# GalDude33/Fetal-MRI-Segmentation

Hardware: NVIDIA B200
Metric: U-Net train voxels/sec (higher is better)
Workload: dtype bf16

## Files before the change

fetal-mri-segmentation_b200/csrc/api.cu:

```cuda
#include <stdarg.h>

#include <algorithm>
#include <cmath>

#include "common.cuh"
#include <chrono>
#include <thread>

static thread_local char g_err[1024] = "";

void fm_set_error(const char* fmt, ...) {
  va_list ap;
  va_start(ap, fmt);
  vsnprintf(g_err, sizeof(g_err), fmt, ap);
  va_end(ap);
}
extern "C" const char* fm_last_error(void) { return g_err; }

extern "C" int fm_ctx_create(int device, fm_ctx** out) {
  FM_CHECK(out != nullptr, FM_EINVAL, "fm_ctx_create: out is NULL");
  int count = 0;
  FM_CUDA(cudaGetDeviceCount(&count));
  FM_CHECK(device >= 0 && device < count, FM_EINVAL, "fm_ctx_create: device %d of %d", device, count);
  FM_CUDA(cudaSetDevice(device));
// ... 810 lines not shown
      if (d < D - 1) {
        FM_TRY(m->gPool[d].ensure((size_t)m->vox(d + 1) * cap * lb.cout));
        const Layer &da = L(m, "dec%da", d), &db = L(m, "dec%db", d);
        if (!da.up_coarse && !da.up_dgrad) FM_TRY(m->gUp[d].ensure(v * da.c1));
        if (m->deconvolution) FM_TRY(m->dcG.ensure(v * da.c1));
        FM_TRY(m->gSkip[d].ensure(v * da.c2));
        FM_TRY(m->gDecA[d].ensure(v * da.cout));
        FM_TRY(m->gDecB[d].ensure(v * db.cout));
      }
    }
    m->train_alloc = true;
  }
  m->cap = cap;
  return FM_OK;
}

static int conv_fwd(fm_model* m, const Layer& l, const bf16* x1, const bf16* x2, bf16* y, int B, int relu = 1) {
  fm_ctx* ctx = m->ctx;
  const Dims5 d = m->dims(l.level, l.cout, B);
  const float* bias = m->params + l.b_off;
  if (l.march_f)
    return k_conv3d_march(ctx, x1, x2, l.w_mf[0], l.w_mf[1], bias, y, nullptr, B, d.X, d.Y, d.Z, l.c1, l.c2, l.cout, relu,
                          l.cout, 0, reproducible_pass(m));
  if (conv_tc_supported(l.c1, l.c2, l.cout, l.k))
    return k_conv3d_tc_fprop(ctx, x1, x2, l.w_f, bias, y, nullptr, B, d.X, d.Y, d.Z, l.c1, l.c2, l.cout,
                             l.k, relu, l.cout, 0);
  return k_conv3d_simt_fprop(ctx, x1, 0, x2, l.w_f, bias, y, nullptr, B, d.X, d.Y, d.Z, l.c1, l.c2,
                             l.cout, l.k, relu, nullptr);
}

static int bn_block_fwd(fm_model* m, const Layer& l, const void* x1, int x1_f32, const bf16* x2, bf16* y, int B) {
  fm_ctx* ctx = m->ctx;
  const int li = (int)(&l - &m->layers[0]);
  const Layer &nl = m->layers[li + 1], &ml = m->layers[li + 2];
  const Dims5 d = m->dims(l.level, l.cout, B);
  bf16* raw = m->train_pass ? m->bnRawL[li + 1].p : m->bnRaw.p;
  if (x1_f32)
    FM_TRY(k_conv3d_simt_fprop(ctx, x1, 1, nullptr, l.w_f, m->params + l.b_off, raw, nullptr, B, d.X, d.Y, d.Z, l.c1, 0,
                               l.cout, l.k, 0, nullptr));
  else
    FM_TRY(conv_fwd(m, l, (const bf16*)x1, x2, raw, B, 0));
  return k_batchnorm_relu(ctx, raw, m->params + nl.w_off, m->params + nl.b_off, m->params + ml.w_off,
                          m->params + ml.b_off, y, B, m->vox(l.level), l.cout, m->bnScratch.p, m->bnScratch.n,
                          m->train_pass ? m->bnStatsL[li + 1].p : nullptr, m->train_pass ? 1 : 0);
}

// ... 136 lines not shown
      FM_TRY(k_conv3d_tc_wgrad(ctx, xs[s], dy, dw, B, d.X, d.Y, d.Z, cs[s], l.cin(), cofs, l.cout, l.k));
    else
      FM_TRY(k_conv3d_simt_wgrad(ctx, xs[s], 0, dy, dw, B, d.X, d.Y, d.Z, cs[s], l.cin(), cofs, l.cout,
                                 l.k));
    cofs += cs[s];
  }
  if (!bias_done) FM_TRY(k_bias_grad(ctx, dy, m->grads + l.b_off, d.voxels(), l.cout));
  return FM_OK;
}

static int conv_wgrad_source(fm_model* m, const Layer& l, int src, const bf16* x, const bf16* dy, int B) {
  return conv_wgrad(m, l, src == 0 ? x : nullptr, src == 1 ? x : nullptr, dy, B, src);
}

static int conv_dgrad(fm_model* m, const Layer& l, int src, const bf16* dy, const bf16* mask, bf16* dx,
                      int B) {
  fm_ctx* ctx = m->ctx;
  const Dims5 d = m->dims(l.level, l.cout, B);
  const int cs = src == 0 ? l.c1 : l.c2;
  const bf16* wd = src == 0 ? l.w_d0 : l.w_d1;
  if (l.march_d[src])
    return k_conv3d_march(ctx, dy, nullptr, l.w_md[src], nullptr, nullptr, dx, mask, B, d.X, d.Y, d.Z, l.cout, 0, cs, 0,
                          cs, 0, reproducible_pass(m));
  if (conv_tc_supported(l.cout, 0, cs, l.k))
    return k_conv3d_tc_fprop(ctx, dy, nullptr, wd, nullptr, dx, mask, B, d.X, d.Y, d.Z, l.cout, 0, cs, l.k,
                             0, cs, 0);
  return k_conv3d_simt_fprop(ctx, dy, 0, nullptr, wd, nullptr, dx, nullptr, B, d.X, d.Y, d.Z, l.cout, 0,
                             cs, l.k, 0, mask);
}

static int mark_layer_done(fm_model* m, const Layer& l) {
  const int i = (int)(&l - &m->layers[0]);
  FM_CUDA(cudaEventRecord(m->layer_done[i], m->ctx->stream));
  return FM_OK;
}

static int backward_isensee(fm_model* m, int B);

static int bn_block_bwd(fm_model* m, const Layer& l, const bf16* gy, const bf16* gy2, int B) {
  const int li = (int)(&l - &m->layers[0]);
  const Layer& nl = m->layers[li + 1];
  FM_TRY(k_batchnorm_relu_bwd(m->ctx, m->bnRawL[li + 1].p, m->bnStatsL[li + 1].p, m->params + nl.w_off,
                              m->params + nl.b_off, gy, gy2, m->bnGRaw.p, m->grads + nl.w_off, m->grads + nl.b_off, B,
                              m->vox(l.level), l.cout, m->bnScratch.p, m->bnScratch.n));
  FM_TRY(mark_layer_done(m, m->layers[li + 2]));
  return mark_layer_done(m, nl);
// ... 380 lines not shown
      FM_TRY(m->isLoc1[l].ensure(n));
      FM_TRY(m->isLoc2[l].ensure(n));
      if (l < m->nseg) FM_TRY(m->isSeg[l].ensure((size_t)B * m->vox(l)));
    }
  }
  m->cap = B;
  return FM_OK;
}

static int isensee_block(fm_model* m, const Layer& l, const Layer& nl, const bf16* x1, const bf16* x2, const bf16* add,
                         bf16* y, int B, const float* chan_scale = nullptr) {
  fm_ctx* ctx = m->ctx;
  const Dims5 d = m->dims(l.level, l.cout, B);
  const float* bias = m->params + l.b_off;
  const int li = (int)(&l - &m->layers[0]);
  bf16* raw = m->train_pass ? m->isRawL[li].p : m->isRaw.p;
  float* stats = m->train_pass ? m->isStatsL[li].p : nullptr;
  if (l.c1 == 1) {
    FM_TRY(k_conv3d_simt_fprop(ctx, x1, 1, nullptr, l.w_f, bias, raw, nullptr, B, d.X, d.Y, d.Z, 1, 0, l.cout, 3, 0,
                               nullptr));
  } else if (l.march_f) {
    FM_TRY(k_conv3d_march(ctx, x1, x2, l.w_mf[0], l.w_mf[1], bias, raw, nullptr, B, d.X, d.Y, d.Z, l.c1, l.c2, l.cout, 0,
                          l.cout, 0, reproducible_pass(m)));
  } else if (conv_tc_supported(l.c1, l.c2, l.cout, l.k)) {
    FM_TRY(k_conv3d_tc_fprop(ctx, x1, x2, l.w_f, bias, raw, nullptr, B, d.X, d.Y, d.Z, l.c1, l.c2, l.cout, l.k, 0,
                             l.cout, 0, l.stride, d.X * l.stride, d.Y * l.stride, m->pz == 2 ? d.Z * l.stride : d.Z));
  } else {
    FM_CHECK(l.stride == 1, FM_EINVAL, "isensee: strided conv %s has no fallback", l.name);
    FM_TRY(k_conv3d_simt_fprop(ctx, x1, 0, x2, l.w_f, bias, raw, nullptr, B, d.X, d.Y, d.Z, l.c1, l.c2, l.cout, l.k, 0,
                               nullptr));
  }
  return k_instnorm_lrelu(ctx, raw, m->params + nl.w_off, m->params + nl.b_off, add, y, B, m->vox(l.level), l.cout,
                          m->isScratch.p, m->isScratch.n, stats, chan_scale);
}

static int forward_isensee(fm_model* m, int B) {
  fm_ctx* ctx = m->ctx;
  const int D = m->depth();
  FM_TRY(refresh_packs(m));
  auto LI = [&](const char* fmt, int d) {
    char nm[32];
    snprintf(nm, sizeof(nm), fmt, d);
    return layer_index(m, nm);
  };
  const bf16* cur = nullptr;
  for (int l = 0; l < D; ++l) {
// ... 50 lines not shown
  const bf16* xs[2] = {x1, x2};
  const int cs[2] = {l.c1, l.c2};
  int cofs = 0;
  for (int s = 0; s < (l.c2 ? 2 : 1); ++s) {
    if (conv_wgrad_march_supported(d.X, d.Y, d.Z, cs[s], l.cout, l.k))
      FM_TRY(k_conv3d_wgrad_march(ctx, xs[s], dy, dw, B, d.X, d.Y, d.Z, cs[s], l.cin(), cofs, l.cout));
    else if (conv_tc_supported(cs[s], 0, l.cout, l.k))
      FM_TRY(k_conv3d_tc_wgrad(ctx, xs[s], dy, dw, B, d.X, d.Y, d.Z, cs[s], l.cin(), cofs, l.cout, l.k));
    else
      FM_TRY(k_conv3d_simt_wgrad(ctx, xs[s], 0, dy, dw, B, d.X, d.Y, d.Z, cs[s], l.cin(), cofs, l.cout, l.k));
    cofs += cs[s];
  }
  return FM_OK;
}

static int is_dgrad(fm_model* m, const Layer& l, int level, int src, const bf16* dy, bf16* dx, int B) {
  fm_ctx* ctx = m->ctx;
  const Dims5 d = m->dims(level, l.cout, B);
  const int cs = src == 0 ? l.c1 : l.c2;
  const bf16* wd = src == 0 ? l.w_d0 : l.w_d1;
  if (l.march_d[src])
    return k_conv3d_march(ctx, dy, nullptr, l.w_md[src], nullptr, nullptr, dx, nullptr, B, d.X, d.Y, d.Z, l.cout, 0, cs, 0,
                          cs, 0, reproducible_pass(m));
  if (conv_tc_supported(l.cout, 0, cs, l.k))
    return k_conv3d_tc_fprop(ctx, dy, nullptr, wd, nullptr, dx, nullptr, B, d.X, d.Y, d.Z, l.cout, 0, cs, l.k, 0, cs, 0);
  return k_conv3d_simt_fprop(ctx, dy, 0, nullptr, wd, nullptr, dx, nullptr, B, d.X, d.Y, d.Z, l.cout, 0, cs, l.k, 0,
                             nullptr);
}

static int is_block_bwd(fm_model* m, int li, const bf16* gy, const bf16* gy2, const float* chan_scale, int B) {
  const Layer &l = m->layers[li], &nl = m->layers[li + 1];
  FM_TRY(k_instnorm_lrelu_bwd(m->ctx, m->isRawL[li].p, m->isStatsL[li].p, m->params + nl.w_off, m->params + nl.b_off, gy,
                              gy2, chan_scale, m->gIsRaw.p, m->grads + nl.w_off, m->grads + nl.b_off, B, m->vox(l.level),
                              l.cout, m->isScratch.p, m->isScratch.n));
  FM_TRY(mark_layer_done(m, nl));
  return FM_OK;
}

static int backward_isensee(fm_model* m, int B) {
  fm_ctx* ctx = m->ctx;
  const int D = m->depth();
  const int64_t n0 = (int64_t)B * m->vox(0);
  auto LI = [&](const char* fmt, int d) {
    char nm[32];
    snprintf(nm, sizeof(nm), fmt, d);
    return layer_index(m, nm);
// ... 927 lines not shown
  OpScratch s(ctx);
  const size_t vox = (size_t)N * X * Y * Z;
  const int taps = kext_taps(ksize), Ct = C1 + C2;
  std::vector<float> packed((size_t)Cout * taps * Ct);
  keras_to_packed(w_keras, packed.data(), ksize, Ct, Cout);
  bf16 *dx1 = nullptr, *dx2 = nullptr, *dw = nullptr, *dy = nullptr;
  float* dbias = nullptr;
  FM_TRY(s.up_bf16(x, vox * C1, &dx1));
  if (C2 > 0) FM_TRY(s.up_bf16(x2, vox * C2, &dx2));
  FM_TRY(s.up_bf16(packed.data(), packed.size(), &dw));
  if (bias) FM_TRY(s.up_f32(bias, Cout, &dbias));
  FM_TRY(s.alloc(&dy, vox * Cout));
  if (impl == 2 || impl == 3) {
    FM_CHECK(conv_march_supported(X, Y, Z, C1, C2, Cout, ksize), FM_EINVAL, "march kernel does not cover this shape");
    bf16 *wm1 = nullptr, *wm2 = nullptr;
    FM_TRY(s.alloc(&wm1, (size_t)conv_march_pack_elems(C1, Cout)));
    FM_TRY(k_repack_march(ctx, dw, wm1, Cout, Ct, 0, C1, conv_march_kc(C1, C2, Cout, C1)));
    if (C2 > 0) {
      FM_TRY(s.alloc(&wm2, (size_t)conv_march_pack_elems(C2, Cout)));
      FM_TRY(k_repack_march(ctx, dw, wm2, Cout, Ct, C1, C2, conv_march_kc(C1, C2, Cout, C2)));
    }
    FM_TRY(k_conv3d_march(ctx, dx1, dx2, wm1, wm2, dbias, dy, nullptr, N, X, Y, Z, C1, C2, Cout, relu, Cout, 0,
                          impl != 3));
  } else if (impl == 0)
    FM_TRY(k_conv3d_tc_fprop(ctx, dx1, dx2, dw, dbias, dy, nullptr, N, X, Y, Z, C1, C2, Cout, ksize, relu,
                             Cout, 0));
  else
    FM_TRY(k_conv3d_simt_fprop(ctx, dx1, 0, dx2, dw, dbias, dy, nullptr, N, X, Y, Z, C1, C2, Cout, ksize,
                               relu, nullptr));
  return s.down_bf16(dy, vox * Cout, y);
}

extern "C" int fm_op_conv3d_dgrad(fm_ctx* ctx, int impl, const float* dy, const float* w_keras,
                                  const float* mask, int N, int X, int Y, int Z, int Cin, int Cout,
                                  float* dx) {
  FM_CHECK(ctx && dy && w_keras && dx, FM_EINVAL, "fm_op_conv3d_dgrad: NULL argument");
  FM_CUDA(cudaSetDevice(ctx->device));
  OpScratch s(ctx);
  const size_t vox = (size_t)N * X * Y * Z;
  const int ksize = 3, taps = 27;
  std::vector<float> packed((size_t)Cout * taps * Cin);
  keras_to_packed(w_keras, packed.data(), ksize, Cin, Cout);
  float* dwm = nullptr;
  bf16 *wd = nullptr, *ddy = nullptr, *dmask = nullptr, *ddx = nullptr;
  FM_TRY(s.up_f32(packed.data(), packed.size(), &dwm));
  FM_TRY(s.alloc(&wd, packed.size()));
  FM_TRY(k_repack_weights(ctx, dwm, nullptr, wd, nullptr, Cout, taps, Cin, 0));
  FM_TRY(s.up_bf16(dy, vox * Cout, &ddy));
  if (mask) FM_TRY(s.up_bf16(mask, vox * Cin, &dmask));
  FM_TRY(s.alloc(&ddx, vox * Cin));
  if (impl == 2 || impl == 3) {
    FM_CHECK(conv_march_supported(X, Y, Z, Cout, 0, Cin, ksize), FM_EINVAL, "march kernel does not cover this shape");
    bf16* wm = nullptr;
    FM_TRY(s.alloc(&wm, (size_t)conv_march_pack_elems(Cout, Cin)));
    FM_TRY(k_repack_march(ctx, wd, wm, Cin, Cout, 0, Cout, conv_march_kc(Cout, 0, Cin, Cout)));
    FM_TRY(k_conv3d_march(ctx, ddy, nullptr, wm, nullptr, nullptr, ddx, dmask, N, X, Y, Z, Cout, 0, Cin, 0, Cin, 0,
                          impl != 3));
  } else if (impl == 0)
    FM_TRY(k_conv3d_tc_fprop(ctx, ddy, nullptr, wd, nullptr, ddx, dmask, N, X, Y, Z, Cout, 0, Cin, ksize, 0,
                             Cin, 0));
  else
    FM_TRY(k_conv3d_simt_fprop(ctx, ddy, 0, nullptr, wd, nullptr, ddx, nullptr, N, X, Y, Z, Cout, 0, Cin,
                               ksize, 0, dmask));
  return s.down_bf16(ddx, vox * Cin, dx);
}

extern "C" int fm_op_conv3d_wgrad(fm_ctx* ctx, int impl, const float* x, const float* dy, int N, int X,
                                  int Y, int Z, int Cin, int Cout, float* dw_keras, float* dbias) {
  FM_CHECK(ctx && x && dy && dw_keras, FM_EINVAL, "fm_op_conv3d_wgrad: NULL argument");
  FM_CUDA(cudaSetDevice(ctx->device));
  OpScratch s(ctx);
  const size_t vox = (size_t)N * X * Y * Z;
  const int ksize = 3, taps = 27;
  bf16 *dx = nullptr, *ddy = nullptr;
  float *dw = nullptr, *db = nullptr;
  FM_TRY(s.up_bf16(x, vox * Cin, &dx));
  FM_TRY(s.up_bf16(dy, vox * Cout, &ddy));
  const size_t wn = (size_t)Cout * taps * Cin;
  FM_TRY(s.alloc(&dw, wn));
  FM_TRY(s.alloc(&db, Cout));
// ... 232 lines not shown
```

fetal-mri-segmentation_b200/csrc/common.cuh:

```cuda
#pragma once
#include <cuda.h>
#include <cuda_bf16.h>
#include <cuda_runtime.h>
#include <stdint.h>
#include <stdio.h>
#include <stdlib.h>
#include <string.h>

#include <string>
#include <vector>

#include "../../include/fetal_b200.h"

typedef __nv_bfloat16 bf16;

void fm_set_error(const char* fmt, ...);

#define FM_CUDA(expr)                                                                         \
  do {                                                                                        \
    cudaError_t _e = (expr);                                                                  \
    if (_e != cudaSuccess) {                                                                  \
      fm_set_error("%s:%d: %s -> %s", __FILE__, __LINE__, #expr, cudaGetErrorString(_e));     \
      return FM_ECUDA;                                                                        \
    }                                                                                         \
// ... 248 lines not shown
                    int C, double* sums, XentSpec xs = XentSpec());
int k_dice_finalize(fm_ctx*, int nblocks, double n_elems, double* sums);
int k_head_bwd(fm_ctx*, const bf16* x, const float* dz, const float* w, bf16* dx, float* dw,
               float* db, int64_t voxels, int C, int mode = 0, const float* t = nullptr, const double* sums = nullptr,
               XentSpec xs = XentSpec());
struct RepackDesc {
  int64_t w_off;
  int cout, taps, c1, c2;
  bf16 *wf, *wd0, *wd1, *mf0, *mf1, *md0, *md1;
  int kcf0, kcf1, kcd0, kcd1;
  int block0;
};
int k_repack_all(fm_ctx*, const float* params, const RepackDesc* table_dev, int nlayers, int total_blocks,
                 double total_weights);
int k_repack_weights(fm_ctx*, const float* w, bf16* w_f, bf16* w_d0, bf16* w_d1, int Cout, int taps,
                     int C1, int C2);

struct ConvTcPlan;
int conv_tc_supported(int C1, int C2, int Cout, int ksize);
int k_conv3d_tc_fprop(fm_ctx*, const bf16* x1, const bf16* x2, const bf16* w_packed,
                      const float* bias, bf16* y, const bf16* mask, int N, int X, int Y, int Z,
                      int C1, int C2, int Cout, int ksize, int relu, int out_C, int out_cofs, int stride = 1,
                      int Xin = 0, int Yin = 0, int Zin = 0);
int k_conv3d_tc_wgrad(fm_ctx*, const bf16* x, const bf16* dy, float* dw_packed, int N, int X, int Y,
                      int Z, int Cin, int Cin_total, int cin_ofs, int Cout, int ksize);
int conv_up_supported(int X, int Y, int Z, int Cc, int Cs, int Cout);
int k_repack_up(fm_ctx*, const float* w_master, bf16* w_up_f, bf16* w_up_d, int Cout, int Cc, int Ct);
struct RepackUpDesc {
  int64_t w_off;
  bf16 *wf, *wd;
  int cout, cc, ct, block0;
};
struct RepackUpTable {
  RepackUpDesc d[8];
  int n;
};
int k_repack_up_table(fm_ctx*, const float* params, const RepackUpTable& tab);
int k_conv3d_up_fprop(fm_ctx*, const bf16* coarse, const bf16* skip, const bf16* w_up, const bf16* w_packed,
                      const float* bias, bf16* y, int N, int X, int Y, int Z, int Cc, int Cs, int Cout, int relu);
int k_conv3d_up_dgrad(fm_ctx*, const bf16* dy, const bf16* w_up_d, bf16* dcoarse, const bf16* mask, int N, int X,
                      int Y, int Z, int Cout, int Cc);
int k_conv3d_up_wgrad(fm_ctx*, const bf16* coarse, const bf16* dy, float* dw_up, int N, int X, int Y, int Z, int Cc,
                      int Cout);
int k_fold_up_wgrad(fm_ctx*, const float* dw_up, float* dw_master, int Cout, int Cc, int Ct);

int conv_first_tc_supported(int X, int Y, int Z, int Cout);
// ... 16 lines not shown
```

fetal-mri-segmentation_b200/csrc/conv_tc.cu:

```cuda
#include <algorithm>

#include "tc_ptx.cuh"

namespace {

using namespace tcp;

constexpr int kTileM = 128;
constexpr int kThreadsTc = 192;
constexpr uint32_t kABytes = kTileM * 128;

struct alignas(64) FpropParams {
  CUtensorMap tmA[2];
  CUtensorMap tmW[2];
  int nsrc;
  int nchunks[2];
  int KC[2];
  int wcofs[2];
  int N, X, Y, Z;
  int bx, by, bz, tx, ty, tz;
  int m_tiles, n_tiles, block_n;
  int ksize, ntaps;
  int out_C, out_cofs;
  int relu;
  int stages;
  int stride;
  int stride_z;
  int pbx, pby, pbz;
  int upmode;
  int ntaps_s[2];
  int oX, oY, oZ;
  const float* bias;
  bf16* out;
  const bf16* mask;
};

__global__ void __launch_bounds__(kThreadsTc, 1) conv3d_tc_fprop_kernel(
    const __grid_constant__ FpropParams p) {
  extern __shared__ uint8_t smem_raw[];
  const uint32_t smem0 = (smem_u32(smem_raw) + 1023u) & ~1023u;
  const int warp = threadIdx.x >> 5, lane = threadIdx.x & 31;

  const uint32_t b_bytes = (uint32_t)p.block_n * 128u;
  const uint32_t stage_bytes = kABytes + b_bytes;
  const uint32_t bar0 = smem0 + (uint32_t)p.stages * stage_bytes;
  auto full_bar = [&](int s) { return bar0 + 8u * (uint32_t)s; };
  auto empty_bar = [&](int s) { return bar0 + 8u * (uint32_t)(p.stages + s); };
  auto tfull_bar = [&](int a) { return bar0 + 8u * (uint32_t)(2 * p.stages + a); };
  auto tempty_bar = [&](int a) { return bar0 + 8u * (uint32_t)(2 * p.stages + 2 + a); };
  const uint32_t tmem_slot = bar0 + 8u * (uint32_t)(2 * p.stages + 4);

  uint32_t tmem_cols = 32;
  while (tmem_cols < 2u * (uint32_t)p.block_n) tmem_cols <<= 1;

  if (warp == 0 && lane == 0) {
    for (int s = 0; s < p.nsrc; ++s) {
      prefetch_tmap(&p.tmA[s]);
      prefetch_tmap(&p.tmW[s]);
// ... 147 lines not shown
      int m = tile / p.n_tiles;
      int cls = 0;
      if (p.upmode == 1) {
        cls = m & 7;
        m >>= 3;
      }
      const int iz = m % p.tz;
      m /= p.tz;
      const int iy = m % p.ty;
      m /= p.ty;
      const int ix = m % p.tx;
      const int n = m / p.tx;
      int x = ix * p.bx + rx, y = iy * p.by + ry, z = iz * p.bz + rz;
      const bool valid = (x < p.X) && (y < p.Y) && (z < p.Z);
      if (p.upmode == 1) {
        x = 2 * x + (cls >> 2);
        y = 2 * y + ((cls >> 1) & 1);
        z = 2 * z + (cls & 1);
      }
      const int64_t v = (((int64_t)n * p.oX + x) * p.oY + y) * p.oZ + z;
      const int64_t off = v * p.out_C + p.out_cofs + n_tile * p.block_n;
      mbar_wait(tfull_bar(acc), acc_ph);
      tc_fence_after();
      const uint32_t taddr = tmem_base + ((uint32_t)(q * 32) << 16) + acc * (uint32_t)p.block_n;
      for (int c16 = 0; c16 < p.block_n / 16; ++c16) {
        uint32_t r[16];
        tmem_ld16(taddr + (uint32_t)c16 * 16u, r);
        tmem_ld_wait();
        if (valid) {
          float f[16];
#pragma unroll
          for (int j = 0; j < 16; ++j) f[j] = __uint_as_float(r[j]);
          if (p.bias != nullptr) {
            const float4* bp =
                reinterpret_cast<const float4*>(p.bias + n_tile * p.block_n + c16 * 16);
#pragma unroll
            for (int j = 0; j < 4; ++j) {
              const float4 b4 = __ldg(bp + j);
              f[4 * j] += b4.x;
              f[4 * j + 1] += b4.y;
              f[4 * j + 2] += b4.z;
              f[4 * j + 3] += b4.w;
            }
          }
          if (p.relu) {
#pragma unroll
            for (int j = 0; j < 16; ++j) f[j] = fmaxf(f[j], 0.f);
          }
          if (p.mask != nullptr) {
            const uint4* mp = reinterpret_cast<const uint4*>(p.mask + off + c16 * 16);
#pragma unroll
            for (int h = 0; h < 2; ++h) {
              const uint4 mv = __ldg(mp + h);
              const __nv_bfloat162* mh = reinterpret_cast<const __nv_bfloat162*>(&mv);
#pragma unroll
              for (int j = 0; j < 4; ++j) {
                const float2 mf = __bfloat1622float2(mh[j]);
                if (!(mf.x > 0.f)) f[8 * h + 2 * j] = 0.f;
                if (!(mf.y > 0.f)) f[8 * h + 2 * j + 1] = 0.f;
              }
            }
          }
          uint4 o[2];
          __nv_bfloat162* oh = reinterpret_cast<__nv_bfloat162*>(o);
#pragma unroll
          for (int j = 0; j < 8; ++j) oh[j] = __floats2bfloat162_rn(f[2 * j], f[2 * j + 1]);
          uint4* op = reinterpret_cast<uint4*>(p.out + off + c16 * 16);
          op[0] = o[0];
          op[1] = o[1];
        }
      }
      tc_fence_before();
      mbar_arrive(tempty_bar(acc));
    }
  }

  tc_fence_before();
  __syncthreads();
  if (warp == 1) {
    tc_fence_after();
    tmem_dealloc(tmem_base, tmem_cols);
  }
}

struct alignas(64) WgradParams {
  CUtensorMap tmX;
  CUtensorMap tmDY;
  int KC, NC;
  int g;
  int ngroups;
  int G;
  int n_gsub;
  int n_cchunks;
  int n_nblocks;
  int NB;
  int splits;
// ... 226 lines not shown
  FM_CHECK(r == CUDA_SUCCESS, FM_ECUDA, "cuTensorMapEncodeTiled(weights) failed: %d (Cout=%d taps=%d Ct=%d)",
           (int)r, Cout, taps, Ct);
  return FM_OK;
}

int pow2_ceil(int v) {
  int p = 1;
  while (p < v) p <<= 1;
  return p;
}

void choose_box(int X, int Y, int Z, int* bx, int* by, int* bz) {
  int z = std::min(kTileM, pow2_ceil(Z));
  int y = std::min(kTileM / z, pow2_ceil(Y));
  int x = kTileM / (z * y);
  *bz = z;
  *by = y;
  *bx = x;
}

bool chan_ok(int C) { return C > 0 && C % 16 == 0 && (C <= 64 ? (C == 16 || C == 32 || C == 64) : C % 64 == 0); }
int chunk_of(int C) { return std::min(C, 64); }


}

int conv_tc_supported(int C1, int C2, int Cout, int ksize) {
  if (!(ksize == 1 || ksize == 3 || ksize == 31)) return 0;
  if (!chan_ok(C1)) return 0;
  if (C2 != 0 && !chan_ok(C2)) return 0;
  if (!(Cout == 16 || Cout == 32 || Cout == 64 || (Cout >= 128 && Cout % 128 == 0))) return 0;
  return 1;
}

int k_conv3d_tc_fprop(fm_ctx* ctx, const bf16* x1, const bf16* x2, const bf16* w_packed,
                      const float* bias, bf16* y, const bf16* mask, int N, int X, int Y, int Z, int C1,
                      int C2, int Cout, int ksize, int relu, int out_C, int out_cofs, int stride, int Xin,
                      int Yin, int Zin) {
  FM_CHECK(stride == 1 || (stride == 2 && kext_xy(ksize) == 3 && C2 == 0), FM_EINVAL,
           "conv3d tc: stride %d unsupported", stride);
  const int stride_z = kext_z(ksize) == 1 ? 1 : stride;
  if (stride == 1) {
    Xin = X;
    Yin = Y;
    Zin = Z;
  }
  FM_CHECK(conv_tc_supported(C1, C2, Cout, ksize), FM_EINVAL,
           "conv3d tc: unsupported channels C1=%d C2=%d Cout=%d k=%d", C1, C2, Cout, ksize);
  FM_CHECK(out_C % 8 == 0 && out_cofs % 8 == 0, FM_EINVAL, "conv3d tc: output channel pitch/offset");
  FpropParams p;
  memset(&p, 0, sizeof(p));
  p.nsrc = C2 > 0 ? 2 : 1;
  p.N = N;
  p.X = X;
  p.Y = Y;
  p.Z = Z;
  choose_box(X, Y, Z, &p.bx, &p.by, &p.bz);
  p.tx = ceil_div(X, p.bx);
  p.ty = ceil_div(Y, p.by);
  p.tz = ceil_div(Z, p.bz);
  p.m_tiles = N * p.tx * p.ty * p.tz;
  p.block_n = std::min(Cout, 128);
  while (p.block_n > 32 && p.m_tiles * (Cout / p.block_n) * 2 <= ctx->num_sms) p.block_n /= 2;
  p.n_tiles = Cout / p.block_n;
  p.ksize = ksize;
  p.ntaps = kext_taps(ksize);
  p.out_C = out_C;
  p.out_cofs = out_cofs;
  p.relu = relu;
  p.bias = bias;
  p.out = y;
  p.mask = mask;
  p.stride = stride;
  p.stride_z = stride_z;
  p.upmode = 0;
  p.ntaps_s[0] = p.ntaps_s[1] = p.ntaps;
  p.oX = X;
  p.oY = Y;
  p.oZ = Z;
  {
    auto pb = [&](int out, int in, int k, int st) { return std::max((out - 1) * st + k - in, 0) / 2; };
    p.pbx = pb(X, Xin, kext_xy(ksize), stride);
    p.pby = pb(Y, Yin, kext_xy(ksize), stride);
    p.pbz = pb(Z, Zin, kext_z(ksize), stride_z);
  }
  const int Ct = C1 + C2;
// ... 4 lines not shown
    p.KC[s] = chunk_of(Cs[s]);
    p.nchunks[s] = Cs[s] / p.KC[s];
    p.wcofs[s] = cofs;
    FM_TRY(make_act_tmap(&p.tmA[s], xs[s], N, Xin, Yin, Zin, Cs[s], p.KC[s], p.bz, p.by, p.bx, stride, stride_z));
    FM_TRY(make_w_tmap(&p.tmW[s], w_packed, Cout, p.ntaps, Ct, p.KC[s], p.block_n));
    cofs += Cs[s];
  }
  const uint32_t stage_bytes = kABytes + (uint32_t)p.block_n * 128u;
  int stages = (kMaxDynSmem - 2048) / (int)stage_bytes;
  stages = std::max(2, std::min(stages, 8));
  p.stages = stages;
  const size_t smem = (size_t)stages * stage_bytes + 1024  + 256 ;
  static bool attr_set = false;
  if (!attr_set) {
    FM_CUDA(cudaFuncSetAttribute(conv3d_tc_fprop_kernel, cudaFuncAttributeMaxDynamicSharedMemorySize,
                                 kMaxDynSmem));
    attr_set = true;
  }
  const int grid = std::min(p.m_tiles * p.n_tiles, ctx->num_sms);
  const double vox = (double)N * X * Y * Z;
  ProfScope prof(ctx, mask != nullptr || bias == nullptr ? "conv3d_tc_dgrad" : "conv3d_tc_fprop",
                 2.0 * p.ntaps * Ct * Cout * vox, vox * (Ct + Cout) * 2.0);
  FM_CUDA(launch_pdl(conv3d_tc_fprop_kernel, dim3(grid), dim3(kThreadsTc), smem, ctx->stream, p));
  FM_LAUNCH_OK(ctx);
  return FM_OK;
}

namespace {

int launch_tc_fprop(fm_ctx* ctx, FpropParams& p, const char* name, double flops, double bytes) {
  const uint32_t stage_bytes = kABytes + (uint32_t)p.block_n * 128u;
  int stages = (kMaxDynSmem - 2048) / (int)stage_bytes;
  stages = std::max(2, std::min(stages, 8));
  p.stages = stages;
  const size_t smem = (size_t)stages * stage_bytes + 1024  + 256 ;
  static bool attr_set = false;
  if (!attr_set) {
    FM_CUDA(cudaFuncSetAttribute(conv3d_tc_fprop_kernel, cudaFuncAttributeMaxDynamicSharedMemorySize, kMaxDynSmem));
    attr_set = true;
  }
  const int grid = std::min(p.m_tiles * p.n_tiles, ctx->num_sms);
  ProfScope prof(ctx, name, flops, bytes);
  FM_CUDA(launch_pdl(conv3d_tc_fprop_kernel, dim3(grid), dim3(kThreadsTc), smem, ctx->stream, p));
  FM_LAUNCH_OK(ctx);
  return FM_OK;
}
// ... 295 lines not shown
```

Before: 656.1 million.

## Add halo-slab tcgen05 3x3x3 conv kernel reusing X-planes across taps

Adds a new tensor-core conv kernel for 3x3x3 stride-1 convolutions. It loads one halo slab (18x10 voxels by 64 channels) per X-plane through TMA and reuses that slab across all nine ky/kz taps and neighbouring X outputs, instead of fetching a separate A tile for every tap. Two X-tiles accumulate in TMEM per work item, and the epilogue is factored into a shared helper. The kernel is routed into fprop, dgrad and isensee forward paths when the shapes fit. It only covers Y%16 and Z%8 shapes with 64-multiple channels, and the slab buffers reduce the number of weight pipeline stages.

```diff
diff --git a/fetal-mri-segmentation_b200/csrc/api.cu b/fetal-mri-segmentation_b200/csrc/api.cu
--- a/fetal-mri-segmentation_b200/csrc/api.cu
+++ b/fetal-mri-segmentation_b200/csrc/api.cu
@@ -856,6 +856,8 @@
   if (l.march_f)
     return k_conv3d_march(ctx, x1, x2, l.w_mf[0], l.w_mf[1], bias, y, nullptr, B, d.X, d.Y, d.Z, l.c1, l.c2, l.cout, relu,
                           l.cout, 0, reproducible_pass(m));
+  if (conv_halo_supported(d.X, d.Y, d.Z, l.c1, l.c2, l.cout, l.k))
+    return k_conv3d_halo(ctx, x1, x2, l.w_f, bias, y, nullptr, B, d.X, d.Y, d.Z, l.c1, l.c2, l.cout, relu, l.cout, 0);
   if (conv_tc_supported(l.c1, l.c2, l.cout, l.k))
     return k_conv3d_tc_fprop(ctx, x1, x2, l.w_f, bias, y, nullptr, B, d.X, d.Y, d.Z, l.c1, l.c2, l.cout,
                              l.k, relu, l.cout, 0);
@@ -1038,6 +1040,8 @@
   if (l.march_d[src])
     return k_conv3d_march(ctx, dy, nullptr, l.w_md[src], nullptr, nullptr, dx, mask, B, d.X, d.Y, d.Z, l.cout, 0, cs, 0,
                           cs, 0, reproducible_pass(m));
+  if (conv_halo_supported(d.X, d.Y, d.Z, l.cout, 0, cs, l.k))
+    return k_conv3d_halo(ctx, dy, nullptr, wd, nullptr, dx, mask, B, d.X, d.Y, d.Z, l.cout, 0, cs, 0, cs, 0);
   if (conv_tc_supported(l.cout, 0, cs, l.k))
     return k_conv3d_tc_fprop(ctx, dy, nullptr, wd, nullptr, dx, mask, B, d.X, d.Y, d.Z, l.cout, 0, cs, l.k,
                              0, cs, 0);
@@ -1464,6 +1468,8 @@
   } else if (l.march_f) {
     FM_TRY(k_conv3d_march(ctx, x1, x2, l.w_mf[0], l.w_mf[1], bias, raw, nullptr, B, d.X, d.Y, d.Z, l.c1, l.c2, l.cout, 0,
                           l.cout, 0, reproducible_pass(m)));
+  } else if (l.stride == 1 && conv_halo_supported(d.X, d.Y, d.Z, l.c1, l.c2, l.cout, l.k)) {
+    FM_TRY(k_conv3d_halo(ctx, x1, x2, l.w_f, bias, raw, nullptr, B, d.X, d.Y, d.Z, l.c1, l.c2, l.cout, 0, l.cout, 0));
   } else if (conv_tc_supported(l.c1, l.c2, l.cout, l.k)) {
     FM_TRY(k_conv3d_tc_fprop(ctx, x1, x2, l.w_f, bias, raw, nullptr, B, d.X, d.Y, d.Z, l.c1, l.c2, l.cout, l.k, 0,
                              l.cout, 0, l.stride, d.X * l.stride, d.Y * l.stride, m->pz == 2 ? d.Z * l.stride : d.Z));
@@ -1560,6 +1566,8 @@
   if (l.march_d[src])
     return k_conv3d_march(ctx, dy, nullptr, l.w_md[src], nullptr, nullptr, dx, nullptr, B, d.X, d.Y, d.Z, l.cout, 0, cs, 0,
                           cs, 0, reproducible_pass(m));
+  if (conv_halo_supported(d.X, d.Y, d.Z, l.cout, 0, cs, l.k))
+    return k_conv3d_halo(ctx, dy, nullptr, wd, nullptr, dx, nullptr, B, d.X, d.Y, d.Z, l.cout, 0, cs, 0, cs, 0);
   if (conv_tc_supported(l.cout, 0, cs, l.k))
     return k_conv3d_tc_fprop(ctx, dy, nullptr, wd, nullptr, dx, nullptr, B, d.X, d.Y, d.Z, l.cout, 0, cs, l.k, 0, cs, 0);
   return k_conv3d_simt_fprop(ctx, dy, 0, nullptr, wd, nullptr, dx, nullptr, B, d.X, d.Y, d.Z, l.cout, 0, cs, l.k, 0,
@@ -2533,6 +2541,9 @@
     }
     FM_TRY(k_conv3d_march(ctx, dx1, dx2, wm1, wm2, dbias, dy, nullptr, N, X, Y, Z, C1, C2, Cout, relu, Cout, 0,
                           impl != 3));
+  } else if (impl == 4) {
+    FM_CHECK(conv_halo_supported(X, Y, Z, C1, C2, Cout, ksize), FM_EINVAL, "halo kernel does not cover this shape");
+    FM_TRY(k_conv3d_halo(ctx, dx1, dx2, dw, dbias, dy, nullptr, N, X, Y, Z, C1, C2, Cout, relu, Cout, 0));
   } else if (impl == 0)
     FM_TRY(k_conv3d_tc_fprop(ctx, dx1, dx2, dw, dbias, dy, nullptr, N, X, Y, Z, C1, C2, Cout, ksize, relu,
                              Cout, 0));
@@ -2567,6 +2578,9 @@
     FM_TRY(k_repack_march(ctx, wd, wm, Cin, Cout, 0, Cout, conv_march_kc(Cout, 0, Cin, Cout)));
     FM_TRY(k_conv3d_march(ctx, ddy, nullptr, wm, nullptr, nullptr, ddx, dmask, N, X, Y, Z, Cout, 0, Cin, 0, Cin, 0,
                           impl != 3));
+  } else if (impl == 4) {
+    FM_CHECK(conv_halo_supported(X, Y, Z, Cout, 0, Cin, ksize), FM_EINVAL, "halo kernel does not cover this shape");
+    FM_TRY(k_conv3d_halo(ctx, ddy, nullptr, wd, nullptr, ddx, dmask, N, X, Y, Z, Cout, 0, Cin, 0, Cin, 0));
   } else if (impl == 0)
     FM_TRY(k_conv3d_tc_fprop(ctx, ddy, nullptr, wd, nullptr, ddx, dmask, N, X, Y, Z, Cout, 0, Cin, ksize, 0,
                              Cin, 0));
diff --git a/fetal-mri-segmentation_b200/csrc/common.cuh b/fetal-mri-segmentation_b200/csrc/common.cuh
--- a/fetal-mri-segmentation_b200/csrc/common.cuh
+++ b/fetal-mri-segmentation_b200/csrc/common.cuh
@@ -294,6 +294,10 @@
                       const float* bias, bf16* y, const bf16* mask, int N, int X, int Y, int Z,
                       int C1, int C2, int Cout, int ksize, int relu, int out_C, int out_cofs, int stride = 1,
                       int Xin = 0, int Yin = 0, int Zin = 0);
+int conv_halo_supported(int X, int Y, int Z, int C1, int C2, int Cout, int ksize);
+int k_conv3d_halo(fm_ctx*, const bf16* x1, const bf16* x2, const bf16* w_packed, const float* bias, bf16* y,
+                  const bf16* mask, int N, int X, int Y, int Z, int C1, int C2, int Cout, int relu, int out_C,
+                  int out_cofs);
 int k_conv3d_tc_wgrad(fm_ctx*, const bf16* x, const bf16* dy, float* dw_packed, int N, int X, int Y,
                       int Z, int Cin, int Cin_total, int cin_ofs, int Cout, int ksize);
 int conv_up_supported(int X, int Y, int Z, int Cc, int Cs, int Cout);
diff --git a/fetal-mri-segmentation_b200/csrc/conv_tc.cu b/fetal-mri-segmentation_b200/csrc/conv_tc.cu
--- a/fetal-mri-segmentation_b200/csrc/conv_tc.cu
+++ b/fetal-mri-segmentation_b200/csrc/conv_tc.cu
@@ -30,10 +30,61 @@
   int upmode;
   int ntaps_s[2];
   int oX, oY, oZ;
+  int ny, nz;
+  PlaneSplit split;
   const float* bias;
   bf16* out;
   const bf16* mask;
 };
+
+__device__ __forceinline__ void epilogue_row(const FpropParams& p, uint32_t taddr, int n_tile, int64_t off, bool valid) {
+  for (int c16 = 0; c16 < p.block_n / 16; ++c16) {
+    uint32_t r[16];
+    tmem_ld16(taddr + (uint32_t)c16 * 16u, r);
+    tmem_ld_wait();
+    if (valid) {
+      float f[16];
+#pragma unroll
+      for (int j = 0; j < 16; ++j) f[j] = __uint_as_float(r[j]);
+      if (p.bias != nullptr) {
+        const float4* bp = reinterpret_cast<const float4*>(p.bias + n_tile * p.block_n + c16 * 16);
+#pragma unroll
+        for (int j = 0; j < 4; ++j) {
+          const float4 b4 = __ldg(bp + j);
+          f[4 * j] += b4.x;
+          f[4 * j + 1] += b4.y;
+          f[4 * j + 2] += b4.z;
+          f[4 * j + 3] += b4.w;
+        }
+      }
+      if (p.relu) {
+#pragma unroll
+        for (int j = 0; j < 16; ++j) f[j] = fmaxf(f[j], 0.f);
+      }
+      if (p.mask != nullptr) {
+        const uint4* mp = reinterpret_cast<const uint4*>(p.mask + off + c16 * 16);
+#pragma unroll
+        for (int h = 0; h < 2; ++h) {
+          const uint4 mv = __ldg(mp + h);
+          const __nv_bfloat162* mh = reinterpret_cast<const __nv_bfloat162*>(&mv);
+#pragma unroll
+          for (int j = 0; j < 4; ++j) {
+            const float2 mf = __bfloat1622float2(mh[j]);
+            if (!(mf.x > 0.f)) f[8 * h + 2 * j] = 0.f;
+            if (!(mf.y > 0.f)) f[8 * h + 2 * j + 1] = 0.f;
+          }
+        }
+      }
+      uint4 o[2];
+      __nv_bfloat162* oh = reinterpret_cast<__nv_bfloat162*>(o);
+#pragma unroll
+      for (int j = 0; j < 8; ++j) oh[j] = __floats2bfloat162_rn(f[2 * j], f[2 * j + 1]);
+      uint4* op = reinterpret_cast<uint4*>(p.out + off + c16 * 16);
+      op[0] = o[0];
+      op[1] = o[1];
+    }
+  }
+}
 
 __global__ void __launch_bounds__(kThreadsTc, 1) conv3d_tc_fprop_kernel(
     const __grid_constant__ FpropParams p) {
@@ -227,56 +278,191 @@
       const int64_t off = v * p.out_C + p.out_cofs + n_tile * p.block_n;
       mbar_wait(tfull_bar(acc), acc_ph);
       tc_fence_after();
-      const uint32_t taddr = tmem_base + ((uint32_t)(q * 32) << 16) + acc * (uint32_t)p.block_n;
-      for (int c16 = 0; c16 < p.block_n / 16; ++c16) {
-        uint32_t r[16];
-        tmem_ld16(taddr + (uint32_t)c16 * 16u, r);
-        tmem_ld_wait();
-        if (valid) {
-          float f[16];
-#pragma unroll
-          for (int j = 0; j < 16; ++j) f[j] = __uint_as_float(r[j]);
-          if (p.bias != nullptr) {
-            const float4* bp =
-                reinterpret_cast<const float4*>(p.bias + n_tile * p.block_n + c16 * 16);
-#pragma unroll
-            for (int j = 0; j < 4; ++j) {
-              const float4 b4 = __ldg(bp + j);
-              f[4 * j] += b4.x;
-              f[4 * j + 1] += b4.y;
-              f[4 * j + 2] += b4.z;
-              f[4 * j + 3] += b4.w;
+      epilogue_row(p, tmem_base + ((uint32_t)(q * 32) << 16) + acc * (uint32_t)p.block_n, n_tile, off, valid);
+      tc_fence_before();
+      mbar_arrive(tempty_bar(acc));
+    }
+  }
+
+  tc_fence_before();
+  __syncthreads();
+  if (warp == 1) {
+    tc_fence_after();
+    tmem_dealloc(tmem_base, tmem_cols);
+  }
+}
+
+constexpr int kHaloT = 2;
+constexpr uint32_t kHaloSlab = 18u * 10u * 128u;
+constexpr uint32_t kHaloSlot = (kHaloSlab + 1023u) & ~1023u;
+constexpr uint32_t kHaloSlots = 6;
+static_assert(kHaloT == 2, "the MMA warp addresses the slabs of tiles 0 and 1");
+
+__global__ void __launch_bounds__(kThreadsTc, 1) conv3d_halo_kernel(const __grid_constant__ FpropParams p) {
+  extern __shared__ uint8_t smem_raw[];
+  const uint32_t smem0 = (smem_u32(smem_raw) + 1023u) & ~1023u;
+  const int warp = threadIdx.x >> 5, lane = threadIdx.x & 31;
+
+  const uint32_t b_bytes = (uint32_t)p.block_n * 128u;
+  const uint32_t w0 = smem0 + kHaloSlots * kHaloSlot;
+  const uint32_t nst = (uint32_t)p.stages;
+  const uint32_t bar0 = w0 + nst * b_bytes;
+  auto afull = [&](uint32_t s) { return bar0 + 8u * s; };
+  auto aempty = [&](uint32_t s) { return bar0 + 8u * (kHaloSlots + s); };
+  auto wfull = [&](uint32_t s) { return bar0 + 8u * (2u * kHaloSlots + s); };
+  auto wempty = [&](uint32_t s) { return bar0 + 8u * (2u * kHaloSlots + nst + s); };
+  auto tfull = [&](uint32_t a) { return bar0 + 8u * (2u * kHaloSlots + 2u * nst + a); };
+  auto tempty = [&](uint32_t a) { return bar0 + 8u * (2u * kHaloSlots + 2u * nst + 2u + a); };
+  const uint32_t tmem_slot = bar0 + 8u * (2u * kHaloSlots + 2u * nst + 4u);
+
+  const uint32_t acc_cols = (uint32_t)kHaloT * (uint32_t)p.block_n;
+  uint32_t tmem_cols = 32;
+  while (tmem_cols < 2u * acc_cols) tmem_cols <<= 1;
+
+  if (warp == 0 && lane == 0) {
+    for (int s = 0; s < p.nsrc; ++s) {
+      prefetch_tmap(&p.tmA[s]);
+      prefetch_tmap(&p.tmW[s]);
+    }
+  }
+  if (warp == 1) {
+    if (lane == 0) {
+      for (uint32_t s = 0; s < kHaloSlots; ++s) {
+        mbar_init(afull(s), 1);
+        mbar_init(aempty(s), 1);
+      }
+      for (uint32_t s = 0; s < nst; ++s) {
+        mbar_init(wfull(s), 1);
+        mbar_init(wempty(s), 1);
+      }
+      for (uint32_t a = 0; a < 2; ++a) {
+        mbar_init(tfull(a), 1);
+        mbar_init(tempty(a), 128);
+      }
+      fence_barrier_init();
+    }
+    __syncwarp();
+    tmem_alloc(tmem_slot, tmem_cols);
+  }
+  tc_fence_before();
+  __syncthreads();
+  tc_fence_after();
+  uint32_t tmem_base;
+  asm volatile("ld.shared.u32 %0, [%1];" : "=r"(tmem_base) : "r"(tmem_slot));
+
+  auto decode = [&](int it, int& n, int& n_tile, int& iy, int& iz, int& xa, int& xb) -> bool {
+    int col;
+    if (!plane_split_next(p.split, (int)blockIdx.x, (int)gridDim.x, it, col, xa, xb)) return false;
+    n_tile = col % p.n_tiles;
+    col /= p.n_tiles;
+    iz = col % p.nz;
+    col /= p.nz;
+    iy = col % p.ny;
+    n = col / p.ny;
+    return true;
+  };
+
+  tmem_base = __shfl_sync(0xffffffffu, tmem_base, 0);
+  const int warp_u = __shfl_sync(0xffffffffu, warp, 0);
+
+  if (warp_u == 0) {
+    pdl_wait();
+    pdl_launch_dependents();
+    uint32_t ws = 0, wph = 0, pc = 0;
+    for (int it = 0, n, n_tile, iy, iz, xa, xb; decode(it, n, n_tile, iy, iz, xa, xb); ++it) {
+      const int nt = xb - xa;
+      const int y0 = iy * 16 - 1, z0 = iz * 8 - 1;
+      for (int s = 0; s < p.nsrc; ++s) {
+        for (int ch = 0; ch < p.nchunks[s]; ++ch) {
+          int tap = 0;
+          for (int kx = 0; kx < 3; ++kx) {
+            for (int j = kx == 0 ? 0 : nt - 1 + kx; j <= nt - 1 + kx; ++j, ++pc) {
+              const uint32_t slot = pc % kHaloSlots;
+              mbar_wait(aempty(slot), ((pc / kHaloSlots) & 1u) ^ 1u);
+              mbar_expect_tx_elect(afull(slot), kHaloSlab);
+              tma_load_5d_elect(smem0 + slot * kHaloSlot, &p.tmA[s], afull(slot), ch * 64, z0, y0, xa - 1 + j, n);
             }
-          }
-          if (p.relu) {
-#pragma unroll
-            for (int j = 0; j < 16; ++j) f[j] = fmaxf(f[j], 0.f);
-          }
-          if (p.mask != nullptr) {
-            const uint4* mp = reinterpret_cast<const uint4*>(p.mask + off + c16 * 16);
-#pragma unroll
-            for (int h = 0; h < 2; ++h) {
-              const uint4 mv = __ldg(mp + h);
-              const __nv_bfloat162* mh = reinterpret_cast<const __nv_bfloat162*>(&mv);
-#pragma unroll
-              for (int j = 0; j < 4; ++j) {
-                const float2 mf = __bfloat1622float2(mh[j]);
-                if (!(mf.x > 0.f)) f[8 * h + 2 * j] = 0.f;
-                if (!(mf.y > 0.f)) f[8 * h + 2 * j + 1] = 0.f;
+            for (int t9 = 0; t9 < 9; ++t9, ++tap) {
+              mbar_wait(wempty(ws), wph ^ 1u);
+              mbar_expect_tx_elect(wfull(ws), b_bytes);
+              tma_load_3d_elect(w0 + ws * b_bytes, &p.tmW[s], wfull(ws), p.wcofs[s] + ch * 64, tap, n_tile * p.block_n);
+              if (++ws == nst) {
+                ws = 0;
+                wph ^= 1u;
               }
             }
           }
-          uint4 o[2];
-          __nv_bfloat162* oh = reinterpret_cast<__nv_bfloat162*>(o);
+        }
+      }
+    }
+  } else if (warp_u == 1) {
+    const uint32_t idesc = make_idesc(kTileM, p.block_n, 0, 0);
+    const uint32_t a_hi = desc_hi(10u * 128u, layout_code(128)), b_hi = desc_hi(8u * 128u, layout_code(128));
+    const uint32_t a_lo0 = desc_lo(smem0, 16u), b_lo0 = desc_lo(w0, 16u);
+    uint32_t ws = 0, wph = 0, pc = 0, ucount = 0;
+    for (int it = 0, n, n_tile, iy, iz, xa, xb; decode(it, n, n_tile, iy, iz, xa, xb); ++it, ++ucount) {
+      const int nt = xb - xa;
+      const uint32_t acc = ucount & 1u, acc_ph = (ucount >> 1) & 1u;
+      mbar_wait(tempty(acc), acc_ph ^ 1u);
+      tc_fence_after();
+      const uint32_t d0 = tmem_base + acc * acc_cols;
+      uint32_t accumulate = 0;
+      for (int s = 0; s < p.nsrc; ++s) {
+        for (int ch = 0; ch < p.nchunks[s]; ++ch) {
+          for (int kx = 0; kx < 3; ++kx) {
+            for (int j = kx == 0 ? 0 : nt - 1 + kx; j <= nt - 1 + kx; ++j) {
+              const uint32_t q = pc + (uint32_t)j;
+              mbar_wait(afull(q % kHaloSlots), (q / kHaloSlots) & 1u);
+            }
+            tc_fence_after();
+            const uint32_t a_t0 = a_lo0 + ((pc + (uint32_t)kx) % kHaloSlots) * (kHaloSlot >> 4);
+            const uint32_t a_t1 = a_lo0 + ((pc + (uint32_t)kx + 1u) % kHaloSlots) * (kHaloSlot >> 4);
+            for (int ky = 0; ky < 3; ++ky) {
+              for (int kz = 0; kz < 3; ++kz) {
+                mbar_wait(wfull(ws), wph);
+                tc_fence_after();
+                const uint32_t b_lo = b_lo0 + ws * (b_bytes >> 4);
+                const uint32_t row16 = (uint32_t)(ky * 10 + kz) * 8u;
+                for (int t = 0; t < nt; ++t) {
+                  const uint32_t a_lo = (t == 0 ? a_t0 : a_t1) + row16;
+                  const uint32_t d_tmem = d0 + (uint32_t)t * (uint32_t)p.block_n;
 #pragma unroll
-          for (int j = 0; j < 8; ++j) oh[j] = __floats2bfloat162_rn(f[2 * j], f[2 * j + 1]);
-          uint4* op = reinterpret_cast<uint4*>(p.out + off + c16 * 16);
-          op[0] = o[0];
-          op[1] = o[1];
+                  for (int k = 0; k < 4; ++k)
+                    umma_bf16_lh_elect(d_tmem, a_lo + 2u * (uint32_t)k, a_hi, b_lo + 2u * (uint32_t)k, b_hi, idesc,
+                                       k == 0 ? accumulate : 1u);
+                }
+                accumulate = 1;
+                umma_commit_elect(wempty(ws));
+                if (++ws == nst) {
+                  ws = 0;
+                  wph ^= 1u;
+                }
+              }
+            }
+            for (int j = kx; j <= (kx == 2 ? nt + 1 : kx); ++j) umma_commit_elect(aempty((pc + (uint32_t)j) % kHaloSlots));
+          }
+          pc += (uint32_t)(nt + 2);
         }
       }
+      umma_commit_elect(tfull(acc));
+    }
+  } else {
+    const int q = warp & 3;
+    const int row = q * 32 + lane;
+    const int yl = row >> 3, zl = row & 7;
+    uint32_t ucount = 0;
+    for (int it = 0, n, n_tile, iy, iz, xa, xb; decode(it, n, n_tile, iy, iz, xa, xb); ++it, ++ucount) {
+      const uint32_t acc = ucount & 1u, acc_ph = (ucount >> 1) & 1u;
+      mbar_wait(tfull(acc), acc_ph);
+      tc_fence_after();
+      for (int t = 0; t < xb - xa; ++t) {
+        const int64_t v = (((int64_t)n * p.X + xa + t) * p.Y + iy * 16 + yl) * p.Z + iz * 8 + zl;
+        const int64_t off = v * p.out_C + p.out_cofs + n_tile * p.block_n;
+        epilogue_row(p, tmem_base + ((uint32_t)(q * 32) << 16) + acc * acc_cols + (uint32_t)(t * p.block_n), n_tile,
+                     off, true);
+      }
       tc_fence_before();
-      mbar_arrive(tempty_bar(acc));
+      mbar_arrive(tempty(acc));
     }
   }
 
@@ -549,6 +735,15 @@
 bool chan_ok(int C) { return C > 0 && C % 16 == 0 && (C <= 64 ? (C == 16 || C == 32 || C == 64) : C % 64 == 0); }
 int chunk_of(int C) { return std::min(C, 64); }
 
+int fprop_block_n(const fm_ctx* ctx, int N, int X, int Y, int Z, int Cout) {
+  int bx, by, bz;
+  choose_box(X, Y, Z, &bx, &by, &bz);
+  const int m_tiles = N * ceil_div(X, bx) * ceil_div(Y, by) * ceil_div(Z, bz);
+  int block_n = std::min(Cout, 128);
+  while (block_n > 32 && m_tiles * (Cout / block_n) * 2 <= ctx->num_sms) block_n /= 2;
+  return block_n;
+}
+
 
 }
 
@@ -587,8 +782,7 @@
   p.ty = ceil_div(Y, p.by);
   p.tz = ceil_div(Z, p.bz);
   p.m_tiles = N * p.tx * p.ty * p.tz;
-  p.block_n = std::min(Cout, 128);
-  while (p.block_n > 32 && p.m_tiles * (Cout / p.block_n) * 2 <= ctx->num_sms) p.block_n /= 2;
+  p.block_n = fprop_block_n(ctx, N, X, Y, Z, Cout);
   p.n_tiles = Cout / p.block_n;
   p.ksize = ksize;
   p.ntaps = kext_taps(ksize);
@@ -639,6 +833,74 @@
   ProfScope prof(ctx, mask != nullptr || bias == nullptr ? "conv3d_tc_dgrad" : "conv3d_tc_fprop",
                  2.0 * p.ntaps * Ct * Cout * vox, vox * (Ct + Cout) * 2.0);
   FM_CUDA(launch_pdl(conv3d_tc_fprop_kernel, dim3(grid), dim3(kThreadsTc), smem, ctx->stream, p));
+  FM_LAUNCH_OK(ctx);
+  return FM_OK;
+}
+
+int conv_halo_supported(int X, int Y, int Z, int C1, int C2, int Cout, int ksize) {
+  if (ksize != 3 || X < 1 || Y < 16 || Y % 16 != 0 || Z < 8 || Z % 8 != 0) return 0;
+  if (C1 <= 0 || C1 % 64 != 0 || C2 < 0 || C2 % 64 != 0) return 0;
+  return Cout == 64 || (Cout >= 128 && Cout % 128 == 0);
+}
+
+int k_conv3d_halo(fm_ctx* ctx, const bf16* x1, const bf16* x2, const bf16* w_packed, const float* bias, bf16* y,
+                  const bf16* mask, int N, int X, int Y, int Z, int C1, int C2, int Cout, int relu, int out_C,
+                  int out_cofs) {
+  FM_CHECK(conv_halo_supported(X, Y, Z, C1, C2, Cout, 3), FM_EINVAL,
+           "conv3d halo: unsupported shape %dx%dx%d C1=%d C2=%d Cout=%d", X, Y, Z, C1, C2, Cout);
+  FM_CHECK(out_C % 8 == 0 && out_cofs % 8 == 0, FM_EINVAL, "conv3d halo: output channel pitch/offset");
+  FpropParams p;
+  memset(&p, 0, sizeof(p));
+  p.nsrc = C2 > 0 ? 2 : 1;
+  p.N = N;
+  p.X = p.oX = X;
+  p.Y = p.oY = Y;
+  p.Z = p.oZ = Z;
+  p.ny = Y / 16;
+  p.nz = Z / 8;
+  p.block_n = fprop_block_n(ctx, N, X, Y, Z, Cout);
+  p.n_tiles = Cout / p.block_n;
+  p.ksize = 3;
+  p.ntaps = 27;
+  p.ntaps_s[0] = p.ntaps_s[1] = 27;
+  p.out_C = out_C;
+  p.out_cofs = out_cofs;
+  p.relu = relu;
+  p.bias = bias;
+  p.out = y;
+  p.mask = mask;
+  p.stride = p.stride_z = 1;
+  const int Ct = C1 + C2;
+  const int Cs[2] = {C1, C2};
+  const bf16* xs[2] = {x1, x2};
+  int cofs = 0;
+  for (int s = 0; s < p.nsrc; ++s) {
+    p.KC[s] = 64;
+    p.nchunks[s] = Cs[s] / 64;
+    p.wcofs[s] = cofs;
+    FM_TRY(make_act_tmap(&p.tmA[s], xs[s], N, X, Y, Z, Cs[s], 64, 10, 18, 1));
+    FM_TRY(make_w_tmap(&p.tmW[s], w_packed, Cout, 27, Ct, 64, p.block_n));
+    cofs += Cs[s];
+  }
+  const int b_bytes = p.block_n * 128;
+  const int slabs = (int)(kHaloSlots * kHaloSlot);
+  p.stages = std::min((kMaxDynSmem - 2048 - slabs) / b_bytes, 16);
+  const size_t smem = (size_t)slabs + (size_t)p.stages * b_bytes + 1024  + 1024 ;
+  static bool attr_set = false;
+  if (!attr_set) {
+    FM_CUDA(cudaFuncSetAttribute(conv3d_halo_kernel, cudaFuncAttributeMaxDynamicSharedMemorySize, kMaxDynSmem));
+    attr_set = true;
+  }
+  const int cols = N * p.n_tiles * p.ny * p.nz;
+  p.split.X = X;
+  p.split.cols = cols;
+  p.split.xchunk = kHaloT;
+  p.split.nxc = ceil_div(X, kHaloT);
+  const int grid = std::min(cols * p.split.nxc, ctx->num_sms);
+  const double vox = (double)N * X * Y * Z;
+  ProfScope prof(ctx, mask != nullptr || bias == nullptr ? "conv3d_halo_dgrad" : "conv3d_halo_fprop",
+                 2.0 * 27 * Ct * Cout * vox, vox * (Ct + Cout) * 2.0);
+  FM_CUDA(launch_pdl(conv3d_halo_kernel, dim3(grid), dim3(kThreadsTc), smem, ctx->stream, p));
   FM_LAUNCH_OK(ctx);
   return FM_OK;
 }
```

Measured after the change: 663.4 million (median of 6 runs). +1.1%, better.
